# kmacrow/Shellac

Measured on AMD Instinct MI355X. Metric: cache_ops_per_s, higher is better.
Workload: dtype uint8

## Files before the change

### shellac_amd/csrc/hbm_cache.h

```cpp
#pragma once

#include <hip/hip_runtime_api.h>

#include <algorithm>
#include <mutex>
#include <string>
#include <vector>

#include "layout.h"

namespace shellac {

enum : int { kEvictFifo = 0, kEvictClock = 1 };

struct ShardConfig {
  uint64_t log_bytes = 1ull << 30;
  uint64_t nbuckets = 1ull << 20;
  uint32_t max_item = 1u << 20;
  int device = 0;
  int evict = kEvictClock;
  uint64_t reinsert_max = 0;
  int serve_blocks = 8;
};

// ... 113 lines not shown
  uint64_t* cur_ring_tail() const { return head_ + 2 + hsel_; }
  uint64_t* next_ring_tail() const { return head_ + 2 + (hsel_ ^ 1); }
  struct RetiredGroup {
    std::vector<void*> ptrs;
    std::vector<hipEvent_t> ev;
    uint64_t bytes = 0;
  };
  void retire_group(std::initializer_list<void*> ptrs, uint64_t bytes, hipStream_t s);
  void reap_retired(bool all);
  void note_stream(hipStream_t s);
  void note_store_end(hipStream_t s);
  std::vector<RetiredGroup> retired_;
  uint64_t retired_ever_ = 0;
  struct SetStream {
    hipStream_t s = nullptr;
    hipEvent_t last = nullptr;
  };
  std::vector<SetStream> set_streams_;
  hipEvent_t ws_ready_ = nullptr;
  hipStream_t ws_grow_stream_ = nullptr;
  std::vector<hipStream_t> ws_ordered_;
  void ws_order(hipStream_t s);
  uint64_t* ring_ = nullptr;
  uint64_t ring_cap_ = 0;
  unsigned long long* rc_ctl_ = nullptr;
  bool lead_ = false;
  bool catch_up_ = true;
  uint64_t rmax_ = 0;
  int64_t rc_cap_ = 0;
  uint64_t *rc_loc_ = nullptr, *rc_h_ = nullptr, *rc_part_ = nullptr, *rc_hx_ = nullptr;
  int64_t rc_adv_w_ = 0;
  struct Pending {
    bool active = false;
    int64_t n = 0, rows = 0, nmove = 0;
    int parity = 0;
    const Digest* keys = nullptr;
    const uint8_t* values = nullptr;
    const uint64_t* voff = nullptr;
    const uint32_t *vlen = nullptr, *flags = nullptr, *expire = nullptr;
    const uint64_t* from = nullptr;
  };
  Pending pend_;
  int hand_b_ = 0;
  struct HandBuf {
    Digest* keys = nullptr;
    uint64_t* voff = nullptr;
    uint64_t* from = nullptr;
    uint32_t *vlen = nullptr, *flags = nullptr, *expire = nullptr;
    int64_t cap = 0;
    uint8_t* scratch = nullptr;
  };
  HandBuf hb_[2];
  struct SetWs {
    uint64_t* dd_keys = nullptr;
    int* dd_win = nullptr;
    uint32_t* dd_slot = nullptr;
    uint64_t *set_size = nullptr, *set_off = nullptr, *set_cnt = nullptr;
    uint32_t* set_claim = nullptr;
  };
  SetWs ws_[2];
  int ws_next_ = 0;
  void select_ws(int p) {
    const SetWs& w = ws_[p];
    dd_keys_ = w.dd_keys; dd_win_ = w.dd_win; dd_slot_ = w.dd_slot; set_size_ = w.set_size;
    set_off_ = w.set_off; set_cnt_ = w.set_cnt; set_claim_ = w.set_claim;
  }

  ShardConfig cfg_;
  uint8_t* log_ = nullptr;
  Entry* index_ = nullptr;
  uint64_t* head_ = nullptr;
  int hsel_ = 0;
  uint64_t* cur_head() const { return head_ + hsel_; }
  uint64_t* claim_ptr() const { return head_ + 4; }
  uint64_t* next_head() const { return head_ + (hsel_ ^ 1); }
  CacheCounters* ctr_ = nullptr;
  unsigned long long* scratch_ = nullptr;
  uint64_t* part_ = nullptr;
  uint64_t* host_buf_ = nullptr;
  uint64_t* host_slots_ = nullptr;
  void* srv_ring_ = nullptr;
  uint64_t* srv_ctl_ = nullptr;
  uint64_t* srv_sync_ = nullptr;
  int srv_blocks_ = 1;
  hipStream_t srv_stream_ = nullptr;
  uint64_t srv_ticket_ = 0, srv_epoch_ = 0, srv_launches_ = 0;
  uint64_t srv_idle_ticks_ = 0, srv_life_ticks_ = 0, srv_khz_ = 0;
  uint64_t* srv_trace_ = nullptr;
  bool srv_running_ = false;
  std::mutex srv_mu_;
  void serve_launch_locked();
  unsigned int* done_ctr_ = nullptr;
  unsigned long long* lb_state_ = nullptr;
  int64_t set_cap_ = 0;
  uint64_t* dd_keys_ = nullptr;
  int* dd_win_ = nullptr;
  uint32_t* dd_slot_ = nullptr;
  uint64_t* set_size_ = nullptr;
  uint64_t* set_off_ = nullptr;
  uint32_t* set_claim_ = nullptr;
  uint64_t* set_cnt_ = nullptr;
  uint32_t dd_mask_ = 0;
  uint64_t ws_gen_ = 0;
  std::mutex mu_;
  hipEvent_t stop_ev_ = nullptr;
  void store_locked(const Digest* keys, const uint8_t* values, const uint64_t* val_off,
                    const uint32_t* vlen, const uint32_t* flags, const uint32_t* expire,
                    int64_t n, uint32_t now, hipStream_t s, hipEvent_t index_after = nullptr,
                    hipEvent_t append_after = nullptr, hipEvent_t append_done = nullptr,
                    const uint64_t* from = nullptr, hipEvent_t plan_done = nullptr,
                    int64_t nmove = 0);
  void store_plan_locked(const Digest* keys, const uint32_t* vlen, int64_t n, hipStream_t s,
                         bool detached = false);
  void store_tail_locked(uint32_t now, hipStream_t s, hipEvent_t index_after,
                         hipEvent_t append_after, hipEvent_t append_done);
  void store_index_locked(const Digest* keys, const uint32_t* vlen, const uint32_t* expire,
                          int64_t n, uint32_t now, hipStream_t s, hipEvent_t index_after,
                          const uint64_t* from = nullptr, int64_t nmove = 0,
                          int win_parity = -1);
};


void device_exclusive_scan(const uint64_t* in, uint64_t* out, int64_t n, void* tmp,
                           size_t tmp_bytes, hipStream_t s);
size_t device_scan_tmp_bytes(int64_t n);

constexpr uint64_t kSegSkip = ~0ull;
void segcopy(const uint8_t* src, const uint64_t* src_off, const uint64_t* dst_off, int64_t n,
             uint8_t* dst, hipStream_t s, uint64_t dst_cap = ~0ull);
void segcopy_dev(const uint64_t* src_off, const uint64_t* dst_off, const int64_t* n_dev,
                 uint8_t* dst, hipStream_t s, uint64_t dst_cap = ~0ull);
void segcopy_sized(const uint8_t* src, const uint64_t* src_off, const uint64_t* dst_off,
                   const uint64_t* seg_len, int64_t n, uint8_t* dst, hipStream_t s,
                   uint64_t cap = ~0ull);

int64_t coalesce_table_slots(int64_t n);
void coalesce_keys(const Digest* keys, int64_t n, uint32_t* table, int64_t table_slots,
                   uint32_t* first, hipStream_t s, uint32_t* cslot = nullptr,
                   bool table_clean = false);
void expand_coalesced(const uint32_t* first, int64_t n, uint64_t* size, uint64_t* off,
                      hipStream_t s);

void expand_coalesced_out(const uint32_t* first, int64_t n, const uint64_t* size,
                          const uint64_t* off, uint64_t* out_size, uint64_t* out_off,
                          uint32_t* table, const uint32_t* cslot, hipStream_t s);

void records_to_set(const uint8_t* rec, const uint64_t* off, const uint64_t* size,
                    const uint64_t* have_size, int64_t n, Digest* keys, uint64_t* val_off,
                    uint32_t* vlen, uint32_t* flags, uint32_t* expire, hipStream_t s);
// ... 16 lines not shown
```

### shellac_amd/csrc/hbm_cache.hip

```cpp
#include <hip/hip_runtime.h>
#include <hip/hip_ext.h>
#include <hipcub/hipcub.hpp>

#include <algorithm>
#include <chrono>
#include <cstdlib>
#include <cstring>
#include <type_traits>
#include <vector>

#include "hbm_cache.h"
#include "trace.h"

namespace shellac {

#define HIP_OK(expr)                                                                   \
  do {                                                                                 \
    hipError_t _e = (expr);                                                            \
    if (_e != hipSuccess)                                                              \
      throw Error(std::string("HIP error ") + hipGetErrorString(_e) + " at " + #expr + \
                  " [" + __FILE__ + ":" + std::to_string(__LINE__) + "]");             \
  } while (0)

namespace {
// ... 1411 lines not shown
      uint64_t* tr = trace + (gticket % kSrvTrace) * 8;
      tr[0] = gticket;
      tr[1] = s_t[0];
      tr[2] = s_t[1];
      tr[3] = t_probed;
      tr[4] = t_copied;
      tr[5] = (uint64_t)wall_clock64();
      tr[6] = (uint64_t)n;
      tr[7] = total;
      __threadfence_system();
      asm volatile("s_waitcnt vmcnt(0)" ::: "memory");
      __hip_atomic_store(slots + s_job[4], total, __ATOMIC_RELEASE, __HIP_MEMORY_SCOPE_SYSTEM);
      __hip_atomic_store(consumed, ticket + 1, __ATOMIC_RELAXED, __HIP_MEMORY_SCOPE_SYSTEM);
      s_t[2] = (uint64_t)wall_clock64();
      if (nblk > 1)
        __hip_atomic_fetch_max(sync, s_t[2], __ATOMIC_RELAXED, __HIP_MEMORY_SCOPE_AGENT);
    }
    ops = wave_sum(ops);
    hits = wave_sum(hits);
    bytes = wave_sum(bytes);
    if (lane == 0) {
      s_cnt[0][w] = ops;
      s_cnt[1][w] = hits;
      s_cnt[2][w] = bytes;
    }
    __syncthreads();
    if (tid == 0) {
      unsigned long long t0 = 0, t1 = 0, t2 = 0;
#pragma unroll
      for (int k = 0; k < kSrvBlock / 64; ++k) {
        t0 += s_cnt[0][k];
        t1 += s_cnt[1][k];
        t2 += s_cnt[2][k];
      }
      CacheCounters* c_ = ctr + (gticket & (kCtrShards - 1));
      if (t0) atomicAdd(&c_->get_ops, t0);
      if (t1) atomicAdd(&c_->get_hits, t1);
      if (t2) atomicAdd(&c_->get_bytes, t2);
    }
    ++ticket;
    __syncthreads();
  }
  if (tid == 0) {
    __hip_atomic_store(consumed, ticket, __ATOMIC_RELAXED, __HIP_MEMORY_SCOPE_SYSTEM);
    const uint64_t out = __hip_atomic_fetch_add(sync + 1, 1ull, __ATOMIC_ACQ_REL,
                                                __HIP_MEMORY_SCOPE_AGENT);
    if (out + 1 == (uint64_t)nblk)
      __hip_atomic_store(ctl + kCtlExited, epoch, __ATOMIC_RELEASE, __HIP_MEMORY_SCOPE_SYSTEM);
  }
}


__global__ __launch_bounds__(kBlock) void k_set_size(const uint32_t* __restrict__ vlen, int64_t n,
                                                     const int* __restrict__ tw,
                                                     const uint32_t* __restrict__ slot_of,
                                                     uint32_t max_item,
                                                     uint64_t* __restrict__ size,
                                                     CacheCounters* __restrict__ ctr,
                                                     uint64_t* __restrict__ part,
                                                     uint64_t* __restrict__ part_cnt) {
  unsigned long long dropped = 0, ops = 0, psum = 0, stored = 0;
  if (blockIdx.x == 0 && threadIdx.x == 0) size[n] = 0;
  const int64_t plen = part_len(n, gridDim.x);
  const int64_t i1 = min(n, (int64_t)(blockIdx.x + 1) * plen);
  for (int64_t i = (int64_t)blockIdx.x * plen + threadIdx.x; i < i1; i += kBlock) {
    if (vlen[i] == kSkipVlen) { size[i] = 0; continue; }
    const bool win = tw[slot_of[i]] == (int)i && vlen[i] <= max_item;
    const uint64_t sz = win ? item_bytes(vlen[i]) : 0;
    size[i] = sz;
    psum += sz;
    ++ops;
    dropped += win ? 0 : 1;
    stored += win ? 1 : 0;
  }
  block_count(ctr, ops, &CacheCounters::set_ops, dropped, &CacheCounters::set_dropped);
  block_partial(psum, part);
  if (part_cnt) block_partial(stored, part_cnt);
}

constexpr uint32_t kClaimDeferred = 0xfffffffeu;

struct Reloc {
  uint64_t alt;
  int target;
};

__device__ __forceinline__ bool copy_entry(Entry* __restrict__ a, uint64_t expect, uint64_t d0,
                                           uint64_t d1, uint64_t loc, uint64_t word) {
  if (atomicCAS(reinterpret_cast<unsigned long long*>(&a->loc), (unsigned long long)expect,
                (unsigned long long)kLockedLoc) != expect)
    return false;
  a->d0 = d0;
  a->d1 = d1;
  *reinterpret_cast<uint64_t*>(&a->vlen) = word;
  __hip_atomic_store(&a->loc, loc, __ATOMIC_RELEASE, __HIP_MEMORY_SCOPE_AGENT);
  return true;
}

__device__ __forceinline__ void drop_entry(Entry* __restrict__ a, uint64_t loc) {
  if (atomicCAS(reinterpret_cast<unsigned long long*>(&a->loc), (unsigned long long)loc,
                (unsigned long long)kLockedLoc) != loc)
    return;
  a->d0 = 0;
  a->d1 = 0;
  __hip_atomic_store(&a->loc, (uint64_t)0, __ATOMIC_RELEASE, __HIP_MEMORY_SCOPE_AGENT);
}
__device__ __forceinline__ Reloc relocate_one(uint64_t p0, uint64_t p1, uint64_t p2, uint64_t p3,
                                         uint64_t r0, uint64_t r1, uint64_t r2, uint64_t r3,
                                         uint64_t b1, uint64_t b2, Entry* __restrict__ index,
                                         uint64_t mask, uint64_t base, uint64_t span,
                                         uint64_t head_new, uint64_t cap, uint32_t now) {
  const int l4 = threadIdx.x & 3;
  const int gbase = threadIdx.x & 60;
  int pick = -1;
  uint64_t a_slot = 0, a_loc = 0;
#pragma unroll 1
  for (int h = 0; h < 2 && pick < 0; ++h) {
    const uint64_t wd0 = h ? r0 : p0, wd1 = h ? r1 : p1, wloc = h ? r2 : p2;
    const uint64_t own = h ? b2 : b1;
    if (wloc - base - 1 < span) continue;
// ... 78 lines not shown
      } else {
        const Reloc r = relocate_one(w1[0], w1[1], w1[2], w1[3], w2[0], w2[1], w2[2], w2[3],
                                     b1, b2, index, mask, base, span, head_new, cap, now);
        target = r.target;
        alt = r.alt;
        if (target == -1) {
          uint64_t oldest = ~0ull;
          target = 0;
#pragma unroll
          for (int e = 0; e < 8; ++e) {
            const uint64_t le = e < 4 ? __shfl(w1[2], gbase + e) : __shfl(w2[2], gbase + e - 4);
            if (le < oldest) { oldest = le; target = e; }
          }
          evict = true;
        }
      }
    }
    if (target < 0) {
      if (attempt == 15 && l4 == 0) ++lost;
      continue;
    }
    const uint64_t e1 = __shfl(w1[2], gbase + (target & 3));
    const uint64_t e2 = __shfl(w2[2], gbase + (target & 3));
    const uint64_t expected = target < 4 ? e1 : e2;
    Entry* const slot = index + (target < 4 ? b1 : b2) * kEntriesPerBucket + (target & 3);
    int ok = 0;
    if (l4 == 0) {
      const unsigned long long prev = atomicCAS(
          reinterpret_cast<unsigned long long*>(&slot->loc), (unsigned long long)expected,
          (unsigned long long)myloc);
      if (prev == expected) {
        slot->d0 = d.lo;
        slot->d1 = d.hi;
        *reinterpret_cast<uint64_t*>(&slot->vlen) = pack2(myvlen, myexp);
        *claim_out = (uint32_t)(slot - index);
        ok = 1;
        evicted += evict ? 1 : 0;
        bytes += myvlen;
      } else if (alt != ~0ull) {
        undo_relocation(index, alt, expected);
      }
    }
    ok = __shfl(ok, gbase);
    if (ok) break;
    if (attempt == 15 && l4 == 0) ++lost;
  }
}

__global__ __launch_bounds__(kBlock) __attribute__((amdgpu_waves_per_eu(8))) void k_set_index(
    const Digest* __restrict__ keys, int64_t n, const uint64_t* __restrict__ size,
    const uint64_t* __restrict__ off, const uint32_t* __restrict__ vlen,
    const uint32_t* __restrict__ expire, Entry* __restrict__ index, uint64_t mask,
    const uint64_t* __restrict__ head_ptr, uint64_t* __restrict__ head_next, uint64_t cap,
    uint32_t now, const uint32_t* __restrict__ slot_of, unsigned long long* __restrict__ dd_keys,
    int* __restrict__ dd_win, CacheCounters* __restrict__ ctr, uint32_t* __restrict__ claim,
    const uint64_t* __restrict__ from, int64_t r0, int64_t r1,
    const unsigned long long* __restrict__ r1_dev) {
  if (r1_dev && (int64_t)*r1_dev < r1) r1 = (int64_t)*r1_dev;
  const int l4 = threadIdx.x & 3;
  const int gbase = threadIdx.x & 60;
  const uint64_t base = *head_ptr;
  const uint64_t head_new = base + off[n];
  const int64_t ngroups = ((int64_t)gridDim.x * kBlock) >> 2;
  unsigned long long evicted = 0, bytes = 0, lost = 0, moved_away = 0;
  if (blockIdx.x == 0 && threadIdx.x == 0) *head_next = head_new;
  for (int64_t i = r0 + (((int64_t)blockIdx.x * kBlock + threadIdx.x) >> 2); i < r1; i += ngroups) {
    if (l4 == 0 && vlen[i] != kSkipVlen) {
      const uint32_t sl = slot_of[i];
      dd_keys[sl] = 0ull;
      dd_win[sl] = -1;
    }
    if (l4 == 0) claim[i] = ~0u;
    if (size[i] == 0) continue;
    const Digest d = keys[i];
    const uint64_t myloc = base + off[i] + 1;
    const uint32_t myvlen = vlen[i];
    const uint32_t myexp = expire ? expire[i] : 0u;
    const uint64_t fr = from ? from[i] : 0ull;
    const uint64_t b1 = bucket1(d, mask), b2 = bucket2(d, mask);
    const uint64_t* q1 = reinterpret_cast<const uint64_t*>(index + b1 * kEntriesPerBucket + l4);
    const uint64_t* q2 = reinterpret_cast<const uint64_t*>(index + b2 * kEntriesPerBucket + l4);
    for (int attempt = 0; attempt < 16; ++attempt) {
      uint64_t w1[4], w2[4];
#pragma unroll
      for (int k = 0; k < 4; ++k) {
        w1[k] = __hip_atomic_load(q1 + k, __ATOMIC_RELAXED, __HIP_MEMORY_SCOPE_AGENT);
        w2[k] = __hip_atomic_load(q2 + k, __ATOMIC_RELAXED, __HIP_MEMORY_SCOPE_AGENT);
      }
      const uint64_t span = head_new - base;
      const bool in1 = w1[2] - base - 1 < span || w1[2] == kLockedLoc;
      const bool in2 = w2[2] - base - 1 < span || w2[2] == kLockedLoc;
      const bool m1 = w1[0] == d.lo && w1[1] == d.hi && !in1;
      const bool m2 = w2[0] == d.lo && w2[1] == d.hi && !in2;
      const bool v1 = !entry_free(w1[2], (uint32_t)(w1[3] >> 32), head_new, cap, now);
      const bool v2 = !entry_free(w2[2], (uint32_t)(w2[3] >> 32), head_new, cap, now);
      const uint32_t mmask = (uint32_t)((__ballot(m1) >> gbase) & 0xfull) |
                             ((uint32_t)((__ballot(m2) >> gbase) & 0xfull) << 4);
      const uint32_t lmask = (uint32_t)((__ballot(v1) >> gbase) & 0xfull) |
                             ((uint32_t)((__ballot(v2) >> gbase) & 0xfull) << 4);
      int target;
      if (fr) {
        const uint32_t fmask = (uint32_t)((__ballot(w1[2] == fr) >> gbase) & 0xfull) |
                               ((uint32_t)((__ballot(w2[2] == fr) >> gbase) & 0xfull) << 4);
        if (!fmask) {
          if (l4 == 0) ++moved_away;
          break;
        }
        target = __ffs(fmask) - 1;
      } else if (mmask) {
        target = __ffs(mmask) - 1;
      } else {
        const uint32_t dead = ~lmask & 0xffu;
        if (dead) {
          const int live1 = __popc(lmask & 0xfu), live2 = __popc(lmask & 0xf0u);
          const uint32_t pref = __popc(dead & 0x0fu) >= 2
                                    ? (dead & 0x0fu)
                                    : (live2 < live1 ? (dead & 0xf0u) : (dead & 0x0fu));
          target = __ffs(pref ? pref : dead) - 1;
        } else {
          if (l4 == 0) claim[i] = kClaimDeferred;
          break;
        }
      }
      const uint64_t e1 = __shfl(w1[2], gbase + (target & 3));
// ... 82 lines not shown
      if (!target && victim) {
        target = victim;
        expected = oldest;
        evict = true;
      }
    }
    if (!target) continue;
    if (copy_entry(target, expected, d.lo, d.hi, myloc, myword)) {
      *claim_out = (uint32_t)(target - index);
      evicted += evict ? 1 : 0;
      bytes += (uint32_t)myword;
      return;
    }
    if (copy) drop_entry(copy, expected);
  }
  ++lost;
}

__global__ __launch_bounds__(kBlock) void k_set_fixup(
    const Digest* __restrict__ keys, int64_t n, const uint64_t* __restrict__ off,
    const uint32_t* __restrict__ vlen, const uint32_t* __restrict__ expire,
    const uint64_t* __restrict__ head_ptr, uint32_t* __restrict__ claim,
    Entry* __restrict__ index, const uint64_t* __restrict__ size, uint64_t* __restrict__ ring,
    uint64_t rmask, const uint64_t* __restrict__ ring_tail, uint64_t* __restrict__ ring_tail_next,
    const uint64_t* __restrict__ cnt_off, uint64_t* __restrict__ head_host, uint64_t mask,
    uint64_t cap, uint32_t now, CacheCounters* __restrict__ ctr) {
  const uint64_t base = *head_ptr;
  const uint64_t rtail = ring ? *ring_tail : 0;
  if (blockIdx.x == 0 && threadIdx.x == 0) {
    if (ring) *ring_tail_next = rtail + cnt_off[n];
    if (head_host)
      __hip_atomic_store(head_host, base + off[n], __ATOMIC_RELAXED, __HIP_MEMORY_SCOPE_SYSTEM);
  }
  if (ring)
    for (int64_t i = (int64_t)blockIdx.x * kBlock + threadIdx.x; i < n;
         i += (int64_t)gridDim.x * kBlock)
      if (size[i]) ring[(rtail + cnt_off[i]) & rmask] = base + off[i] + 0;
  unsigned long long evicted = 0, lost = 0, bytes = 0;
  for (int64_t i = (int64_t)blockIdx.x * kBlock + threadIdx.x; i < n;
       i += (int64_t)gridDim.x * kBlock) {
    if (!size[i]) continue;
    uint32_t c = claim[i];
    if (c == kClaimDeferred) {
      claim[i] = ~0u;
      deferred_insert(keys[i], base + off[i] + 1, pack2(vlen[i], expire ? expire[i] : 0u), index,
                      mask, base, off[n], base + off[n], cap, now, claim + i, evicted, bytes,
                      lost);
      continue;
    }
    if (c == ~0u) continue;
    Entry* const e = index + c;
    if (e->loc != base + off[i] + 1) continue;
    const Digest d = keys[i];
    e->d0 = d.lo;
    e->d1 = d.hi;
    *reinterpret_cast<uint64_t*>(&e->vlen) = pack2(vlen[i], expire ? expire[i] : 0u);
  }
  block_count(ctr, evicted, &CacheCounters::set_evicted, lost, &CacheCounters::set_dropped, bytes,
              &CacheCounters::set_bytes);
}

constexpr int kSmallSetRows = kBlock;
constexpr int kSetSmallU = 16;

__global__ __launch_bounds__(kBlock) void k_set_small(
    const Digest* __restrict__ keys, const uint8_t* __restrict__ values,
    const uint64_t* __restrict__ val_off, const uint32_t* __restrict__ vlen,
    const uint32_t* __restrict__ flags, const uint32_t* __restrict__ expire, int n,
    uint32_t max_item, Entry* __restrict__ index, uint64_t mask,
    const uint64_t* __restrict__ head_ptr, uint64_t* __restrict__ head_next,
    unsigned long long* __restrict__ claim_word, uint64_t cap, uint32_t now,
    uint8_t* __restrict__ log, uint64_t* __restrict__ ring, uint64_t rmask,
    const uint64_t* __restrict__ ring_tail, uint64_t* __restrict__ ring_tail_next,
    uint64_t* __restrict__ head_host, CacheCounters* __restrict__ ctr) {
  constexpr int kT = 2 * kSmallSetRows;
  __shared__ unsigned long long s_tk[kT];
  __shared__ int s_tw[kT];
  __shared__ uint64_t s_off[kSmallSetRows + 1];
  __shared__ uint64_t s_src[kSmallSetRows];
  __shared__ uint32_t s_cnt[kSmallSetRows + 1];
  __shared__ uint32_t s_claim[kSmallSetRows];
  __shared__ Digest s_key[kSmallSetRows];
  __shared__ uint32_t s_vl[kSmallSetRows];
  __shared__ uint32_t s_ex[kSmallSetRows];
  __shared__ unsigned long long s_w[2][kBlock / 64];
  const int tid = threadIdx.x, lane = tid & 63, w = tid >> 6;
  for (int k = tid; k < kT; k += kBlock) {
    s_tk[k] = 0ull;
    s_tw[k] = -1;
  }
  __syncthreads();
  const bool row = tid < n;
  const uint32_t vl = row ? vlen[tid] : kSkipVlen;
  const bool skip = vl == kSkipVlen;
  Digest d{0, 0};
  int slot = -1;
  s_vl[tid] = vl;
  s_ex[tid] = row && expire ? expire[tid] : 0u;
  if (row && !skip) {
    d = keys[tid];
    s_key[tid] = d;
    const unsigned long long key = d.lo ? d.lo : 1ull;
    uint32_t t = (uint32_t)fmix64(key) & (kT - 1);
    for (int probe = 0; probe < kT; ++probe) {
      const unsigned long long prev = atomicCAS(&s_tk[t], 0ull, key);
      if (prev == 0ull || prev == key) {
        atomicMax(&s_tw[t], tid);
        slot = (int)t;
        break;
// ... 349 lines not shown
      if (j == a.W - 1) rc_hx[a.W] = hx + h;
    }
  }
  const unsigned long long mb = __ballot(meets);
  if (mb && lane == __ffsll((long long)mb) - 1) atomicMin(&a.ctl[2], (unsigned long long)j);
  block_count(ctr, nre, &CacheCounters::reinserted, bre, &CacheCounters::reinsert_bytes);
}

struct RcAdvance {
  unsigned long long* ctl = nullptr;
  const uint64_t* ring_tail = nullptr;
  uint64_t rmask = 0;
  int64_t W = 0;
  const uint64_t* ring = nullptr;
  const uint64_t* head = nullptr;
  uint64_t cap = 0;
  int catch_up = 1;
};

__device__ __forceinline__ uint64_t hand_catch_up(const uint64_t* ring, uint64_t rmask,
                                                  uint64_t hand, uint64_t rtail, uint64_t head,
                                                  uint64_t cap) {
  auto over = [&](uint64_t idx) {
    const uint64_t l = ring[idx & rmask];
    return l != kRingSkip && head > l + cap;
  };
  if (hand >= rtail || !over(hand)) return hand;
  uint64_t lo = hand + 1, hi = rtail;
  while (lo < hi) {
    const uint64_t mid = lo + (hi - lo) / 2;
    if (over(mid)) lo = mid + 1; else hi = mid;
  }
  return lo;
}

__device__ __forceinline__ void rc_advance(const RcAdvance& r) {
  const uint64_t rtail = *r.ring_tail;
  const uint64_t hand0 = r.ctl[0];
  const uint64_t weff = r.ctl[3];
  const unsigned long long cut = r.ctl[2];
  const uint64_t consumed = cut != ~0ull && cut < weff ? cut : weff;
  uint64_t hand = hand0 + consumed;
  if (rtail - hand > r.rmask + 1) hand = rtail - (r.rmask + 1);
  if (r.catch_up) hand = hand_catch_up(r.ring, r.rmask, hand, rtail, *r.head, r.cap);
  r.ctl[0] = hand;
  r.ctl[1] = 0;
  r.ctl[2] = ~0ull;
  r.ctl[3] = 0;
  r.ctl[4] = consumed;
}

__global__ __launch_bounds__(kBlock) void k_set_dedupe(const Digest* __restrict__ keys,
                                                       const uint32_t* __restrict__ vlen, int64_t n,
                                                       unsigned long long* __restrict__ tk,
                                                       int* __restrict__ tw, uint32_t tmask,
                                                       uint32_t* __restrict__ slot_of,
                                                       RcAdvance adv) {
  if (adv.ctl && blockIdx.x == 0 && threadIdx.x == 0) rc_advance(adv);
  for (int64_t i = (int64_t)blockIdx.x * kBlock + threadIdx.x; i < n;
       i += (int64_t)gridDim.x * kBlock) {
    if (vlen[i] == kSkipVlen) { slot_of[i] = 0; continue; }
    const unsigned long long key = keys[i].lo ? keys[i].lo : 1ull;
    uint32_t s = (uint32_t)fmix64(key) & tmask;
    for (uint32_t probe = 0; probe <= tmask; ++probe) {
      const unsigned long long prev = atomicCAS(&tk[s], 0ull, key);
      if (prev == 0ull || prev == key) {
        atomicMax(&tw[s], (int)i);
        slot_of[i] = s;
        break;
      }
      s = (s + 1) & tmask;
    }
  }
}

__global__ __launch_bounds__(kBlock) void k_delete(const Digest* __restrict__ keys, int64_t n,
                                                   Entry* __restrict__ index, uint64_t mask,
                                                   const uint64_t* __restrict__ head_ptr,
                                                   uint64_t cap, uint32_t now,
                                                   uint8_t* __restrict__ found,
                                                   CacheCounters* __restrict__ ctr) {
  const int l16 = threadIdx.x & 15;
  const uint64_t head = *head_ptr;
  const int64_t ngroups = ((int64_t)gridDim.x * kBlock) >> 4;
  unsigned long long ops = 0, hits = 0;
  for (int64_t i = ((int64_t)blockIdx.x * kBlock + threadIdx.x) >> 4; i < n; i += ngroups) {
    const Digest d = keys[i];
    const uint64_t b = (l16 < 8) ? bucket1(d, mask) : bucket2(d, mask);
    Entry* const bucket = index + b * kEntriesPerBucket;
    const uint4 v = reinterpret_cast<const uint4*>(bucket)[l16 & 7];
    const uint64_t a = pack2(v.x, v.y), c = pack2(v.z, v.w);
    const uint64_t pa = __shfl_xor(a, 1), pc = __shfl_xor(c, 1);
    const bool even = (l16 & 1) == 0;
    int was_live = 0;
    if (even && a == d.lo && c == d.hi && pa != 0) {
      Entry* const slot = bucket + ((l16 & 7) >> 1);
      const unsigned long long prev =
          atomicCAS(reinterpret_cast<unsigned long long*>(&slot->loc), (unsigned long long)pa, 0ull);
      if (prev == pa && entry_live(pa, (uint32_t)(pc >> 32), head, cap, now)) was_live = 1;
    }
    const unsigned long long any = __ballot(was_live);
    const int gbase = threadIdx.x & 48;
    const int f = ((any >> gbase) & 0xffffull) != 0;
    if (l16 == 0) {
      ++ops;
      hits += f;
      if (found) found[i] = (uint8_t)f;
    }
  }
  block_count(ctr, ops, &CacheCounters::del_ops, hits, &CacheCounters::del_hits);
}

__global__ __launch_bounds__(kBlock) void k_sweep(Entry* __restrict__ index, uint64_t nslots,
                                                  const uint64_t* __restrict__ head_ptr,
                                                  uint64_t cap, uint32_t now,
                                                  unsigned long long* __restrict__ out,
                                                  CacheCounters* __restrict__ ctr) {
  const uint64_t head = *head_ptr;
  unsigned long long live = 0, bytes = 0, swept = 0;
  for (uint64_t k = (uint64_t)blockIdx.x * kBlock + threadIdx.x; k < nslots;
// ... 362 lines not shown
  memset(srv_ctl_, 0, kCtlWords * sizeof(uint64_t));
  HIP_OK(hipMalloc(&srv_sync_, 64));
  HIP_OK(hipHostMalloc(&srv_trace_, kSrvTrace * 8 * sizeof(uint64_t),
                       hipHostMallocMapped | hipHostMallocCoherent));
  memset(srv_trace_, 0, kSrvTrace * 8 * sizeof(uint64_t));
  {
    int khz = 0;
    HIP_OK(hipDeviceGetAttribute(&khz, hipDeviceAttributeWallClockRate, cfg_.device));
    if (khz <= 0) khz = 100000;
    srv_khz_ = (uint64_t)khz;
    srv_idle_ticks_ = (uint64_t)khz * kSrvIdleUs / 1000;
    srv_life_ticks_ = (uint64_t)khz * kSrvLifeUs / 1000;
  }
  HIP_OK(hipMemset(index_, 0, cfg_.nbuckets * kBucketBytes));
  HIP_OK(hipMemset(head_, 0, 64));
  HIP_OK(hipMemset(ctr_, 0, kCtrShards * sizeof(CacheCounters)));
  SH_CHECK(cfg_.evict == kEvictFifo || cfg_.evict == kEvictClock, "unknown eviction policy");
  SH_CHECK(cfg_.max_item <= kVlenMask, "max_item must be < 2 GiB (CLOCK bit in vlen)");
  if (cfg_.evict == kEvictClock) {
    rmax_ = reinsert_budget(cfg_.log_bytes, cfg_.reinsert_max);
    ring_cap_ = ring_entries(cfg_.nbuckets);
    HIP_OK(hipMalloc(&ring_, ring_cap_ * sizeof(uint64_t)));
    HIP_OK(hipMalloc(&rc_ctl_, 8 * sizeof(unsigned long long)));
    HIP_OK(hipMemset(rc_ctl_, 0, 8 * sizeof(unsigned long long)));
    HIP_OK(hipMemset(rc_ctl_ + 2, 0xff, sizeof(unsigned long long)));
    for (HandBuf& b : hb_) HIP_OK(hipMalloc(&b.scratch, rmax_ + 64));
  }
  HIP_OK(hipDeviceSynchronize());
}

HbmCache::~HbmCache() {
  DeviceGuard g(cfg_.device);
  try {
    serve_stop();
  } catch (...) {
  }
  (void)hipDeviceSynchronize();
  if (srv_stream_) (void)hipStreamDestroy(srv_stream_);
  (void)hipHostFree(srv_ring_);
  (void)hipHostFree(srv_ctl_);
  (void)hipHostFree(srv_trace_);
  (void)hipFree(srv_sync_);
  (void)hipFree(log_);
  (void)hipFree(index_);
  (void)hipFree(head_);
  (void)hipFree(ctr_);
  (void)hipFree(scratch_);
  (void)hipFree(done_ctr_);
  (void)hipFree(lb_state_);
  (void)hipFree(part_);
  (void)hipHostFree(host_buf_);
  (void)hipHostFree(host_slots_);
  for (SetWs& w : ws_)
    for (void* p : {(void*)w.dd_keys, (void*)w.dd_win, (void*)w.dd_slot, (void*)w.set_size,
                    (void*)w.set_off, (void*)w.set_claim, (void*)w.set_cnt})
      (void)hipFree(p);
  (void)hipFree(ring_); (void)hipFree(rc_ctl_);
  for (void* p : {(void*)rc_loc_, (void*)rc_h_, (void*)rc_part_, (void*)rc_hx_}) (void)hipFree(p);
  for (HandBuf& b : hb_)
    for (void* p : {(void*)b.keys, (void*)b.voff, (void*)b.from, (void*)b.vlen, (void*)b.flags,
                    (void*)b.expire, (void*)b.scratch})
      (void)hipFree(p);
  reap_retired(true);
  if (ws_ready_) (void)hipEventDestroy(ws_ready_);
  for (const SetStream& x : set_streams_)
    if (x.last) (void)hipEventDestroy(x.last);
}

void HbmCache::retire_group(std::initializer_list<void*> ptrs, uint64_t bytes, hipStream_t s) {
  RetiredGroup g;
  for (void* p : ptrs)
    if (p) g.ptrs.push_back(p);
  if (g.ptrs.empty()) return;
  g.bytes = bytes;
  retired_ever_ += bytes;
  for (const SetStream& x : set_streams_)
    if (x.s != s && x.last) HIP_OK(hipStreamWaitEvent(s, x.last, 0));
  hipEvent_t e;
  HIP_OK(hipEventCreateWithFlags(&e, hipEventDisableTiming));
  HIP_OK(hipEventRecord(e, s));
  g.ev.push_back(e);
  retired_.push_back(std::move(g));
}

void HbmCache::reap_retired(bool all) {
  for (size_t i = 0; i < retired_.size();) {
    bool done = true;
    for (hipEvent_t e : retired_[i].ev)
      if (all) (void)hipEventSynchronize(e);
      else if (hipEventQuery(e) != hipSuccess) done = false;
    if (!done) {
      ++i;
      continue;
    }
    for (hipEvent_t e : retired_[i].ev) (void)hipEventDestroy(e);
    for (void* p : retired_[i].ptrs) (void)hipFree(p);
    retired_.erase(retired_.begin() + (long)i);
  }
}

uint64_t HbmCache::retired_bytes() {
  std::lock_guard<std::mutex> lk(mu_);
  DeviceGuard g(cfg_.device);
  reap_retired(false);
  uint64_t b = 0;
  for (const RetiredGroup& r : retired_) b += r.bytes;
  return b;
// ... 56 lines not shown
  HIP_OK(hipMalloc(&h.expire, cap * 4));
  h.cap = cap;
}

bool HbmCache::should_reclaim(uint64_t bytes_bound) const {
  if (cfg_.evict != kEvictClock) return false;
  const uint64_t h = __atomic_load_n(host_slots_ + kHeadSlot, __ATOMIC_ACQUIRE);
  return h + 4 * (bytes_bound + rmax_) > cfg_.log_bytes;
}

void HbmCache::reclaim_locked(const Digest* keys, const uint8_t* values, const uint64_t* val_off,
                              const uint32_t* vlen, const uint32_t* flags, const uint32_t* expire,
                              int64_t n, int64_t w, uint64_t rmax, uint32_t now, hipStream_t s,
                              bool detached, bool lead) {
  RcArgs a{ring_, ring_cap_ - 1, detached ? next_ring_tail() : cur_ring_tail(), rc_ctl_, w, n,
           hand_b_, claim_ptr(), cfg_.log_bytes, now, rmax, lead ? 1ull : 0ull};
  const int g = (int)((w + kBlock - 1) / kBlock);
  const HandBuf& hb = hb_[hand_b_];
  const RcBatch cb{hb.keys, hb.voff, hb.vlen, hb.flags, hb.expire, hb.from};
  static const int rk = [] {
    const char* e = getenv("SHELLAC_RCSCAN_K");
    const int v = e ? atoi(e) : kRcScanK;
    return v == 1 || v == 2 || v == 4 ? v : kRcScanK;
  }();
  const int gk = (g + rk - 1) / rk;
  if (rk == 4)
    hipLaunchKernelGGL(k_rc_scan<4>, dim3(gk), dim3(kBlock), 0, s, a, cb, log_, index_,
                       cfg_.nbuckets - 1, keys, values, val_off, vlen, flags, expire, n,
                       cfg_.max_item, rc_loc_, rc_h_, rc_part_);
  else if (rk == 2)
    hipLaunchKernelGGL(k_rc_scan<2>, dim3(gk), dim3(kBlock), 0, s, a, cb, log_, index_,
                       cfg_.nbuckets - 1, keys, values, val_off, vlen, flags, expire, n,
                       cfg_.max_item, rc_loc_, rc_h_, rc_part_);
  else
    hipLaunchKernelGGL(k_rc_scan<1>, dim3(gk), dim3(kBlock), 0, s, a, cb, log_, index_,
                       cfg_.nbuckets - 1, keys, values, val_off, vlen, flags, expire, n,
                       cfg_.max_item, rc_loc_, rc_h_, rc_part_);
  hipLaunchKernelGGL(k_rc_emit, dim3(g), dim3(kBlock), 0, s, a, cb, log_, rc_loc_, rc_h_,
                     rc_part_, rc_hx_, hb.scratch, ctr_);
  if (!lead)
    launch_segcopy<2>(s, log_, rc_loc_, rc_hx_, w, hb.scratch, nullptr, nullptr, nullptr,
                      nullptr, rc_h_, rmax);
  rc_adv_w_ = w;
  HIP_OK(hipGetLastError());
}

void HbmCache::ensure_set_ws(int64_t n, hipStream_t s) {
  if (n <= set_cap_) return;
  int64_t cap = set_cap_ ? set_cap_ : 1024;
  while (cap < n) cap *= 2;
  const uint64_t tslots = (uint64_t)cap * 2;
  const uint64_t oc = (uint64_t)set_cap_;
  for (SetWs& w : ws_) {
    retire_group({w.dd_keys, w.dd_win, w.dd_slot, w.set_size, w.set_off, w.set_claim, w.set_cnt},
                 2 * oc * 12 + oc * 8 + 3 * (oc + 1) * 8, s);
    HIP_OK(hipMalloc(&w.dd_keys, tslots * sizeof(uint64_t)));
    HIP_OK(hipMalloc(&w.dd_win, tslots * sizeof(int)));
    HIP_OK(hipMemsetAsync(w.dd_keys, 0, tslots * sizeof(uint64_t), s));
    HIP_OK(hipMemsetAsync(w.dd_win, 0xff, tslots * sizeof(int), s));
    HIP_OK(hipMalloc(&w.dd_slot, cap * sizeof(uint32_t)));
    HIP_OK(hipMalloc(&w.set_size, (cap + 1) * sizeof(uint64_t)));
    HIP_OK(hipMalloc(&w.set_off, (cap + 1) * sizeof(uint64_t)));
    HIP_OK(hipMalloc(&w.set_claim, cap * sizeof(uint32_t)));
    HIP_OK(hipMalloc(&w.set_cnt, (cap + 1) * sizeof(uint64_t)));
  }
  select_ws(0);
  dd_mask_ = (uint32_t)(tslots - 1);
  set_cap_ = cap;
  ++ws_gen_;
  if (!ws_ready_) HIP_OK(hipEventCreateWithFlags(&ws_ready_, hipEventDisableTiming));
  HIP_OK(hipEventRecord(ws_ready_, s));
  ws_grow_stream_ = s;
  ws_ordered_.clear();
}

void HbmCache::reserve(int64_t n) {
  std::lock_guard<std::mutex> lk(mu_);
  DeviceGuard g(cfg_.device);
  if (cfg_.evict == kEvictClock && rmax_ && n > 0) {
    const int64_t w = hand_window(n);
    ensure_rc_ws(w, nullptr);
    ensure_cb(0, w + n, nullptr);
    ensure_cb(1, w + n, nullptr);
    n = w + n;
  }
  ensure_set_ws(n, nullptr);
  HIP_OK(hipDeviceSynchronize());
  reap_retired(true);
}

void HbmCache::lookup(const Digest* keys, int64_t n, uint64_t* loc, uint64_t* size, uint64_t* off,
                      uint32_t now, hipStream_t s, uint64_t reserve, int total_slot,
                      const uint32_t* first) {
  TraceRange tr("hbm.lookup");
  SH_CHECK(total_slot < kHostSlots, "host slot out of range");
  std::lock_guard<std::mutex> lk(mu_);
  DeviceGuard g(cfg_.device);
  uint64_t* ht = total_slot >= 0 ? host_slots_ + total_slot : nullptr;
  if (ht) __atomic_store_n(ht, kSlotPending, __ATOMIC_RELEASE);
  if (n <= 0) {
    HIP_OK(hipMemsetAsync(off, 0, sizeof(uint64_t), s));
    if (ht) *ht = 0;
    return;
  }
  const int grid = grid_for(n * 8, kBlock, kMaxGrid);
  hipLaunchKernelGGL(k_probe, dim3(grid), dim3(kBlock), 0, s, keys, n, index_, cfg_.nbuckets - 1,
                     cur_head(), reserve, cfg_.log_bytes, now, loc, size, ctr_, part_, first,
                     (int64_t)1, (const int64_t*)nullptr, (const uint64_t*)nullptr);
  HIP_OK(hipGetLastError());
  launch_offsets(size, n, part_, grid, off, s, ht);
}

// ... 333 lines not shown
    p.vlen = vlen;
    p.flags = flags;
    p.expire = expire;
  }
  ws_order(s);
  select_ws(p.parity);
  store_plan_locked(p.keys, p.vlen, p.rows, s, detached);
  if (plan_done) HIP_OK(hipEventRecord(plan_done, s));
  pend_ = p;
  if (detached) return;
  store_tail_locked(now, s, index_after, append_after, append_done);
}

void HbmCache::store_tail_locked(uint32_t now, hipStream_t s, hipEvent_t index_after,
                                 hipEvent_t append_after, hipEvent_t append_done) {
  const Pending p = pend_;
  pend_.active = false;
  select_ws(p.parity);
  if (append_after) HIP_OK(hipStreamWaitEvent(s, append_after, 0));
  launch_segcopy<1>(s, p.values, p.voff, set_off_, p.rows, log_, p.keys, p.vlen, p.flags,
                    p.expire, cur_head(), cfg_.log_bytes);
  HIP_OK(hipGetLastError());
  if (append_done) HIP_OK(hipEventRecord(append_done, s));
  store_index_locked(p.keys, p.vlen, p.expire, p.rows, now, s, index_after, p.from, p.nmove,
                     p.nmove ? p.parity : -1);
  hsel_ ^= 1;
}

void HbmCache::store_locked(const Digest* keys, const uint8_t* values, const uint64_t* val_off,
                            const uint32_t* vlen, const uint32_t* flags, const uint32_t* expire,
                            int64_t n, uint32_t now, hipStream_t s, hipEvent_t index_after,
                            hipEvent_t append_after, hipEvent_t append_done,
                            const uint64_t* from, hipEvent_t plan_done, int64_t nmove) {
  store_plan_locked(keys, vlen, n, s);
  if (plan_done) HIP_OK(hipEventRecord(plan_done, s));
  if (append_after) HIP_OK(hipStreamWaitEvent(s, append_after, 0));
  launch_segcopy<1>(s, values, val_off, set_off_, n, log_, keys, vlen, flags, expire, cur_head(),
                    cfg_.log_bytes);
  HIP_OK(hipGetLastError());
  if (append_done) HIP_OK(hipEventRecord(append_done, s));
  store_index_locked(keys, vlen, expire, n, now, s, index_after, from, nmove);
}

void HbmCache::store_plan_locked(const Digest* keys, const uint32_t* vlen, int64_t n,
                                 hipStream_t s, bool detached) {
  const int grid = grid_for(n, kBlock, kMaxGrid);
  RcAdvance adv;
  if (rc_adv_w_ > 0) {
    adv = RcAdvance{rc_ctl_, detached ? next_ring_tail() : cur_ring_tail(), ring_cap_ - 1,
                    rc_adv_w_, ring_, claim_ptr(), cfg_.log_bytes, catch_up_ ? 1 : 0};
    rc_adv_w_ = 0;
  }
  hipLaunchKernelGGL(k_set_dedupe, dim3(grid), dim3(kBlock), 0, s, keys, vlen, n,
                     (unsigned long long*)dd_keys_, dd_win_, dd_mask_, dd_slot_, adv);
  const int sgrid = grid_for(n, kBlock, kMaxGrid);
  uint64_t* part_cnt = ring_ ? part_ + 2 * kMaxGrid : nullptr;
  hipLaunchKernelGGL(k_set_size, dim3(sgrid), dim3(kBlock), 0, s, vlen, n, dd_win_, dd_slot_,
                     cfg_.max_item, set_size_, ctr_, part_ + kMaxGrid, part_cnt);
  HIP_OK(hipGetLastError());
  launch_offsets(set_size_, n, part_ + kMaxGrid, sgrid, set_off_, s, nullptr, 0, part_cnt,
                 ring_ ? set_cnt_ : nullptr, detached ? claim_ptr() : cur_head(), claim_ptr());
}

void HbmCache::store_index_locked(const Digest* keys, const uint32_t* vlen,
                                  const uint32_t* expire, int64_t n, uint32_t now, hipStream_t s,
                                  hipEvent_t index_after, const uint64_t* from, int64_t nmove,
                                  int win_parity) {
  if (index_after) HIP_OK(hipStreamWaitEvent(s, index_after, 0));
  if (!from) nmove = 0;
  for (int pass = nmove > 0 ? 0 : 1; pass < 2; ++pass) {
    const int64_t r0 = pass ? nmove : 0, r1 = pass ? n : nmove;
    if (r1 <= r0) continue;
    const int igrid = grid_for((r1 - r0) * 4, kBlock, kMaxGrid);
    hipLaunchKernelGGL(k_set_index, dim3(igrid), dim3(kBlock), 0, s, keys, n, set_size_, set_off_,
                       vlen, expire, index_, cfg_.nbuckets - 1, cur_head(), next_head(),
                       cfg_.log_bytes, now, dd_slot_, (unsigned long long*)dd_keys_, dd_win_,
                       ctr_, set_claim_, pass ? (const uint64_t*)nullptr : from, r0, r1,
                       pass || win_parity < 0 ? nullptr : rc_ctl_ + 5 + win_parity);
  }
  launch_stop(&stop_ev_, k_set_fixup, dim3(grid_for(n, kBlock, kMaxGrid)), dim3(kBlock), s, keys,
              n, set_off_, vlen, expire, cur_head(), set_claim_, index_, set_size_, ring_,
              ring_ ? ring_cap_ - 1 : 0ull, cur_ring_tail(), next_ring_tail(), set_cnt_,
              host_slots_ + kHeadSlot, cfg_.nbuckets - 1, cfg_.log_bytes, now, ctr_);
  HIP_OK(hipGetLastError());
}

void HbmCache::destroy_graph(StoreGraph* g) {
  for (auto& e : g->exec)
    if (e) {
      (void)hipGraphExecDestroy(e);
      e = nullptr;
    }
  g->n = -1;
}

void HbmCache::store_graph(StoreGraph* g, const Digest* keys, const uint8_t* values,
                           const uint64_t* val_off, const uint32_t* vlen, const uint32_t* flags,
                           const uint32_t* expire, int64_t n, uint64_t bytes_bound,
                           uint32_t now, hipStream_t s) {
  TraceRange tr("hbm.store_graph");
  if (n <= 0) return;
  SH_CHECK(s != nullptr, "store_graph needs a created stream (the legacy default stream "
                         "cannot be captured)");
  SH_CHECK(bytes_bound <= cfg_.log_bytes / 2,
           "SET batch larger than half the log; split the batch");
  std::lock_guard<std::mutex> lk(mu_);
  DeviceGuard dg(cfg_.device);
  ensure_set_ws(n, s);
  ws_order(s);
  select_ws(0);
  const void* ptrs[6] = {keys, values, val_off, vlen, flags, expire};
  bool same = g->n == n && g->bound == bytes_bound && g->now == now && g->ws_gen == ws_gen_ &&
              g->exec[0] && g->exec[1];
  for (int i = 0; same && i < 6; ++i) same = g->ptrs[i] == ptrs[i];
  if (!same) {
    destroy_graph(g);
    const int keep = hsel_;
    for (int p = 0; p < 2; ++p) {
      hsel_ = p;
      hipGraph_t graph = nullptr;
      HIP_OK(hipStreamBeginCapture(s, hipStreamCaptureModeRelaxed));
      try {
        store_locked(keys, values, val_off, vlen, flags, expire, n, now, s);
      } catch (...) {
        (void)hipStreamEndCapture(s, &graph);
        if (graph) (void)hipGraphDestroy(graph);
        hsel_ = keep;
        throw;
      }
      HIP_OK(hipStreamEndCapture(s, &graph));
// ... 222 lines not shown
```

Before: 3.474 billion.

## Merge dedupe key and winner tables into one 32-bit index table

Replaces the separate 64-bit key table and int winner table used for in-batch set deduplication with a single uint32 table that stores index+1 of the claiming item. Key comparison now reads the original key from the keys array. This cuts dedupe table memory, memset size and atomic width, and reset writes in k_set_index. The fixup kernel also skips index-entry writes when the stored fields already match. The trade-offs are an extra dependent load on collision and extra reads before the conditional writes in fixup.

```diff
diff --git a/shellac_amd/csrc/hbm_cache.h b/shellac_amd/csrc/hbm_cache.h
--- a/shellac_amd/csrc/hbm_cache.h
+++ b/shellac_amd/csrc/hbm_cache.h
@@ -189,8 +189,7 @@
   };
   HandBuf hb_[2];
   struct SetWs {
-    uint64_t* dd_keys = nullptr;
-    int* dd_win = nullptr;
+    uint32_t* dd_tab = nullptr;
     uint32_t* dd_slot = nullptr;
     uint64_t *set_size = nullptr, *set_off = nullptr, *set_cnt = nullptr;
     uint32_t* set_claim = nullptr;
@@ -199,7 +198,7 @@
   int ws_next_ = 0;
   void select_ws(int p) {
     const SetWs& w = ws_[p];
-    dd_keys_ = w.dd_keys; dd_win_ = w.dd_win; dd_slot_ = w.dd_slot; set_size_ = w.set_size;
+    dd_tab_ = w.dd_tab; dd_slot_ = w.dd_slot; set_size_ = w.set_size;
     set_off_ = w.set_off; set_cnt_ = w.set_cnt; set_claim_ = w.set_claim;
   }
 
@@ -230,8 +229,7 @@
   unsigned int* done_ctr_ = nullptr;
   unsigned long long* lb_state_ = nullptr;
   int64_t set_cap_ = 0;
-  uint64_t* dd_keys_ = nullptr;
-  int* dd_win_ = nullptr;
+  uint32_t* dd_tab_ = nullptr;
   uint32_t* dd_slot_ = nullptr;
   uint64_t* set_size_ = nullptr;
   uint64_t* set_off_ = nullptr;
diff --git a/shellac_amd/csrc/hbm_cache.hip b/shellac_amd/csrc/hbm_cache.hip
--- a/shellac_amd/csrc/hbm_cache.hip
+++ b/shellac_amd/csrc/hbm_cache.hip
@@ -1487,7 +1487,7 @@
 
 
 __global__ __launch_bounds__(kBlock) void k_set_size(const uint32_t* __restrict__ vlen, int64_t n,
-                                                     const int* __restrict__ tw,
+                                                     const uint32_t* __restrict__ tw,
                                                      const uint32_t* __restrict__ slot_of,
                                                      uint32_t max_item,
                                                      uint64_t* __restrict__ size,
@@ -1500,7 +1500,7 @@
   const int64_t i1 = min(n, (int64_t)(blockIdx.x + 1) * plen);
   for (int64_t i = (int64_t)blockIdx.x * plen + threadIdx.x; i < i1; i += kBlock) {
     if (vlen[i] == kSkipVlen) { size[i] = 0; continue; }
-    const bool win = tw[slot_of[i]] == (int)i && vlen[i] <= max_item;
+    const bool win = tw[slot_of[i]] == (uint32_t)i + 1u && vlen[i] <= max_item;
     const uint64_t sz = win ? item_bytes(vlen[i]) : 0;
     size[i] = sz;
     psum += sz;
@@ -1685,8 +1685,8 @@
     const uint64_t* __restrict__ off, const uint32_t* __restrict__ vlen,
     const uint32_t* __restrict__ expire, Entry* __restrict__ index, uint64_t mask,
     const uint64_t* __restrict__ head_ptr, uint64_t* __restrict__ head_next, uint64_t cap,
-    uint32_t now, const uint32_t* __restrict__ slot_of, unsigned long long* __restrict__ dd_keys,
-    int* __restrict__ dd_win, CacheCounters* __restrict__ ctr, uint32_t* __restrict__ claim,
+    uint32_t now, const uint32_t* __restrict__ slot_of, uint32_t* __restrict__ dd_tab,
+    CacheCounters* __restrict__ ctr, uint32_t* __restrict__ claim,
     const uint64_t* __restrict__ from, int64_t r0, int64_t r1,
     const unsigned long long* __restrict__ r1_dev) {
   if (r1_dev && (int64_t)*r1_dev < r1) r1 = (int64_t)*r1_dev;
@@ -1698,11 +1698,7 @@
   unsigned long long evicted = 0, bytes = 0, lost = 0, moved_away = 0;
   if (blockIdx.x == 0 && threadIdx.x == 0) *head_next = head_new;
   for (int64_t i = r0 + (((int64_t)blockIdx.x * kBlock + threadIdx.x) >> 2); i < r1; i += ngroups) {
-    if (l4 == 0 && vlen[i] != kSkipVlen) {
-      const uint32_t sl = slot_of[i];
-      dd_keys[sl] = 0ull;
-      dd_win[sl] = -1;
-    }
+    if (l4 == 0 && vlen[i] != kSkipVlen) dd_tab[slot_of[i]] = 0u;
     if (l4 == 0) claim[i] = ~0u;
     if (size[i] == 0) continue;
     const Digest d = keys[i];
@@ -1891,9 +1887,12 @@
     Entry* const e = index + c;
     if (e->loc != base + off[i] + 1) continue;
     const Digest d = keys[i];
-    e->d0 = d.lo;
-    e->d1 = d.hi;
-    *reinterpret_cast<uint64_t*>(&e->vlen) = pack2(vlen[i], expire ? expire[i] : 0u);
+    uint64_t* const ew = reinterpret_cast<uint64_t*>(&e->vlen);
+    const uint64_t w = pack2(vlen[i], expire ? expire[i] : 0u);
+    const uint64_t e0 = e->d0, e1 = e->d1, e3 = *ew;
+    if (e0 != d.lo) e->d0 = d.lo;
+    if (e1 != d.hi) e->d1 = d.hi;
+    if ((e3 & ~(uint64_t)kRefBit) != w) *ew = w;
   }
   block_count(ctr, evicted, &CacheCounters::set_evicted, lost, &CacheCounters::set_dropped, bytes,
               &CacheCounters::set_bytes);
@@ -2349,8 +2348,7 @@
 
 __global__ __launch_bounds__(kBlock) void k_set_dedupe(const Digest* __restrict__ keys,
                                                        const uint32_t* __restrict__ vlen, int64_t n,
-                                                       unsigned long long* __restrict__ tk,
-                                                       int* __restrict__ tw, uint32_t tmask,
+                                                       uint32_t* __restrict__ tw, uint32_t tmask,
                                                        uint32_t* __restrict__ slot_of,
                                                        RcAdvance adv) {
   if (adv.ctl && blockIdx.x == 0 && threadIdx.x == 0) rc_advance(adv);
@@ -2360,9 +2358,14 @@
     const unsigned long long key = keys[i].lo ? keys[i].lo : 1ull;
     uint32_t s = (uint32_t)fmix64(key) & tmask;
     for (uint32_t probe = 0; probe <= tmask; ++probe) {
-      const unsigned long long prev = atomicCAS(&tk[s], 0ull, key);
-      if (prev == 0ull || prev == key) {
-        atomicMax(&tw[s], (int)i);
+      const uint32_t prev = atomicCAS(&tw[s], 0u, (uint32_t)i + 1u);
+      if (prev == 0u) {
+        slot_of[i] = s;
+        break;
+      }
+      const unsigned long long ok = prev <= (uint32_t)n ? keys[prev - 1].lo : 0ull;
+      if (prev <= (uint32_t)n && (ok ? ok : 1ull) == key) {
+        atomicMax(&tw[s], (uint32_t)i + 1u);
         slot_of[i] = s;
         break;
       }
@@ -2831,7 +2834,7 @@
   (void)hipHostFree(host_buf_);
   (void)hipHostFree(host_slots_);
   for (SetWs& w : ws_)
-    for (void* p : {(void*)w.dd_keys, (void*)w.dd_win, (void*)w.dd_slot, (void*)w.set_size,
+    for (void* p : {(void*)w.dd_tab, (void*)w.dd_slot, (void*)w.set_size,
                     (void*)w.set_off, (void*)w.set_claim, (void*)w.set_cnt})
       (void)hipFree(p);
   (void)hipFree(ring_); (void)hipFree(rc_ctl_);
@@ -2994,12 +2997,10 @@
   const uint64_t tslots = (uint64_t)cap * 2;
   const uint64_t oc = (uint64_t)set_cap_;
   for (SetWs& w : ws_) {
-    retire_group({w.dd_keys, w.dd_win, w.dd_slot, w.set_size, w.set_off, w.set_claim, w.set_cnt},
-                 2 * oc * 12 + oc * 8 + 3 * (oc + 1) * 8, s);
-    HIP_OK(hipMalloc(&w.dd_keys, tslots * sizeof(uint64_t)));
-    HIP_OK(hipMalloc(&w.dd_win, tslots * sizeof(int)));
-    HIP_OK(hipMemsetAsync(w.dd_keys, 0, tslots * sizeof(uint64_t), s));
-    HIP_OK(hipMemsetAsync(w.dd_win, 0xff, tslots * sizeof(int), s));
+    retire_group({w.dd_tab, w.dd_slot, w.set_size, w.set_off, w.set_claim, w.set_cnt},
+                 2 * oc * 4 + oc * 8 + 3 * (oc + 1) * 8, s);
+    HIP_OK(hipMalloc(&w.dd_tab, tslots * sizeof(uint32_t)));
+    HIP_OK(hipMemsetAsync(w.dd_tab, 0, tslots * sizeof(uint32_t), s));
     HIP_OK(hipMalloc(&w.dd_slot, cap * sizeof(uint32_t)));
     HIP_OK(hipMalloc(&w.set_size, (cap + 1) * sizeof(uint64_t)));
     HIP_OK(hipMalloc(&w.set_off, (cap + 1) * sizeof(uint64_t)));
@@ -3439,10 +3440,10 @@
     rc_adv_w_ = 0;
   }
   hipLaunchKernelGGL(k_set_dedupe, dim3(grid), dim3(kBlock), 0, s, keys, vlen, n,
-                     (unsigned long long*)dd_keys_, dd_win_, dd_mask_, dd_slot_, adv);
+                     dd_tab_, dd_mask_, dd_slot_, adv);
   const int sgrid = grid_for(n, kBlock, kMaxGrid);
   uint64_t* part_cnt = ring_ ? part_ + 2 * kMaxGrid : nullptr;
-  hipLaunchKernelGGL(k_set_size, dim3(sgrid), dim3(kBlock), 0, s, vlen, n, dd_win_, dd_slot_,
+  hipLaunchKernelGGL(k_set_size, dim3(sgrid), dim3(kBlock), 0, s, vlen, n, dd_tab_, dd_slot_,
                      cfg_.max_item, set_size_, ctr_, part_ + kMaxGrid, part_cnt);
   HIP_OK(hipGetLastError());
   launch_offsets(set_size_, n, part_ + kMaxGrid, sgrid, set_off_, s, nullptr, 0, part_cnt,
@@ -3461,8 +3462,8 @@
     const int igrid = grid_for((r1 - r0) * 4, kBlock, kMaxGrid);
     hipLaunchKernelGGL(k_set_index, dim3(igrid), dim3(kBlock), 0, s, keys, n, set_size_, set_off_,
                        vlen, expire, index_, cfg_.nbuckets - 1, cur_head(), next_head(),
-                       cfg_.log_bytes, now, dd_slot_, (unsigned long long*)dd_keys_, dd_win_,
-                       ctr_, set_claim_, pass ? (const uint64_t*)nullptr : from, r0, r1,
+                       cfg_.log_bytes, now, dd_slot_, dd_tab_, ctr_, set_claim_,
+                       pass ? (const uint64_t*)nullptr : from, r0, r1,
                        pass || win_parity < 0 ? nullptr : rc_ctl_ + 5 + win_parity);
   }
   launch_stop(&stop_ev_, k_set_fixup, dim3(grid_for(n, kBlock, kMaxGrid)), dim3(kBlock), s, keys,
```

New measurement: 3.610 billion, median of 6. 3.9% higher.
